# Alee08/multiagent-rl-rm

Hardware: AMD Instinct MI355X
Metric: env×agent steps/sec at 65,536 envs (1/2/4/8 GPU) + CPU-ref parity rate (higher is better)
Workload: dtype int32; 1 GPU; FrozenLake map1, 65,536 envs/GPU x 2 agents, built-in A->B->C RM (3-state RM), random actions; n_envs_per_gpu=65536, n_envs_total=65536, n_agents=2, rm_states=4, parallelism=dp1 (env shards, no data-path collective), dispatch=queue, windows=5

## Files before the change

include/rmx.h:

```cpp
#ifndef RMX_H
#define RMX_H

#include <stdint.h>
#include <stddef.h>

#ifdef __cplusplus
extern "C" {
#endif

#define RMX_ABI_VERSION 12

#define RMX_MAX_AGENTS 8
#define RMX_MAX_CELLS 4096
#define RMX_MAX_RM_STATES 255
#define RMX_MAX_EVENTS 255

#define RMX_OK 0
#define RMX_E_INVALID (-1)
#define RMX_E_HIP (-2)
#define RMX_E_ACTION (-3)
#define RMX_E_STATE (-4)
#define RMX_E_TRACE (-5)

#define RMX_DEVICE_HOST (-1)
// ... 106 lines not shown
int rmx_step_hashed(rmx_handle* h, uint64_t seed, int64_t t_global, int autoreset, void* hip_stream);

int rmx_fill_actions(rmx_handle* h, uint64_t seed, int64_t t0, int32_t T, int32_t* actions_dev,
                     void* hip_stream);

int rmx_rollout(rmx_handle* h, uint64_t seed, int64_t t0, int32_t T, float* reward_trace_dev,
                void* hip_stream);

int rmx_mdp_states(rmx_handle* h, int32_t agent, int64_t* n_states);
int rmx_mdp(rmx_handle* h, int32_t agent, int32_t fix_frozen_lake, int32_t* next_dev, float* reward_dev,
            uint8_t* done_dev, void* hip_stream);

int rmx_stats_device(rmx_handle* h, double* out_dev, void* hip_stream);
int rmx_stats_host(rmx_handle* h, double* out_host);
int rmx_stats_clear(rmx_handle* h, void* hip_stream);

int rmx_step_report(rmx_handle* h, const int32_t* actions_dev, int autoreset, double* stats_out_dev,
                    void* hip_stream);
int rmx_step_report_fused(const rmx_handle* h);

int rmx_step_seq(rmx_handle* h, const int32_t* actions_dev, int64_t action_stride, int32_t n_steps, int autoreset,
                 double* stats_out_dev, void* hip_stream);
int rmx_seq_packed(const rmx_handle* h);
int rmx_queue_counters(const rmx_handle* h, int64_t* out3);
#define RMX_QUEUE_INFO_N 7
#define RMX_QUEUE_UNUSED 0
#define RMX_QUEUE_READY 1
#define RMX_QUEUE_UNAVAILABLE 2
#define RMX_QUEUE_RETIRED 3
#define RMX_SEQ_NONE 0
#define RMX_SEQ_QUEUE 1
#define RMX_SEQ_STREAM_KERNEL 2
#define RMX_SEQ_STREAM_DISABLED 3
#define RMX_SEQ_STREAM_QUEUE 4
#define RMX_SEQ_HOST 5
int rmx_queue_info(const rmx_handle* h, int64_t* out, int32_t n);
int rmx_queue_timing(rmx_handle* h, int every);
int rmx_queue_times(const rmx_handle* h, uint64_t* stamps, int64_t cap, int64_t* n);
int rmx_code_object_check(const void* co, size_t bytes, int64_t* n_step_kernels, int64_t* n_refused, char* report,
                          size_t report_cap);

#define RMX_VARIANT_GENERIC 0
#define RMX_VARIANT_LANE_PER_AGENT 1
#define RMX_VARIANT_FAST 2
#define RMX_VARIANT_FAST_LANE_PER_AGENT 3
#define RMX_VARIANT_HOST 4
// ... 58 lines not shown
```

multiagent-rl-rm_amd/csrc/rmx_capi_create.cpp:

```cpp
#include <algorithm>
#include <cstdlib>
#include <cstring>
#include <exception>
#include <string>
#include <vector>

#include "rmx_handle.h"

using namespace rmx::capi;

namespace {

int validate(const rmx_config* c) {
  if (!c) return fail(RMX_E_INVALID, "config is NULL");
  const std::string msg = rmx::validate_config(*c);
  return msg.empty() ? RMX_OK : fail(RMX_E_INVALID, msg);
}

int create_host(const rmx_config* cfg, rmx_handle** out) {
  rmx_handle* h = new rmx_handle();
  h->host = new rmx::HostEngine();
  const std::string msg = h->host->init(*cfg);
  if (!msg.empty()) {
    delete h->host;
// ... 19 lines not shown
      mj *= M;
      const u128 v[2] = {mj, sj};
      for (int k = 0; k < 2; ++k)
        for (int q = 0; q < 4; ++q) w[j][k][q] = (uint32_t)(v[k] >> (32 * q));
    }
  }
};
const RsJumpTable rs_jump_table;

}

extern "C" {

struct CreateTables {
  std::vector<unsigned char> blob, fast_blob;
  std::vector<uint32_t> merged_tab;
  std::vector<float> disc;
  std::vector<uint16_t> free_cells;
};

static void create_env(rmx_handle* h, const rmx_config* cfg) {
  if (const char* qv = std::getenv("RMX_QUEUE")) h->seq.queue_off = std::strcmp(qv, "0") == 0;
  if (const char* pv = std::getenv("RMX_SEQ_PACKED")) h->seq.packed_off = std::strcmp(pv, "0") == 0;
  if (const char* b = std::getenv("RMX_BLOCK")) {
    int v = std::atoi(b);
    if (v == 64 || v == 128 || v == 256) h->block = v;
  }
#ifdef RMX_DIAG
  if (const char* d = std::getenv("RMX_DIAG_BITS")) h->diag = std::atoi(d);
#endif
  const bool rng_on = cfg->stochastic || cfg->random_starts;
  if (rng_on) h->rollout_layout = rmx::kLayoutThreadPerEnv;
  if (const char* l = std::getenv("RMX_LAYOUT")) {
    if (!std::strcmp(l, "tpe")) h->step_layout = h->rollout_layout = rmx::kLayoutThreadPerEnv;
    if (!std::strcmp(l, "lpe") && !rng_on) h->step_layout = h->rollout_layout = rmx::kLayoutLanePerAgent;
  }
}

static bool create_plan(rmx_handle* h, const rmx_config* cfg, CreateTables& tb) {
  const int A = cfg->n_agents;
  for (int a = 0; a < A; ++a) {
    h->init_q[a] = cfg->init_q[a];
    h->final_q[a] = cfg->final_q[a];
    h->start_x[a] = cfg->start_xy[2 * a];
    h->start_y[a] = cfg->start_xy[2 * a + 1];
  }
// ... 170 lines not shown
```

multiagent-rl-rm_amd/csrc/rmx_capi_seq.cpp:

```cpp
#include <algorithm>
#include <atomic>
#include <cstring>
#include <exception>

#include "rmx_handle.h"

using namespace rmx::capi;

static bool seq_packs(const rmx_handle* h) {
  const int tm = h->fast_tables;
  return !h->seq.packed_off && !h->seq.pk_failed && !h->seq.pk_refused && h->cfg.n_envs < kFastWaveStatsMinEnvs &&
         rmx::pk_bytes(h->cfg.n_agents, (size_t)h->cfg.n_envs) < ((size_t)1 << 31) && fast_applies(h) && !h->cfg.stochastic && !h->cfg.random_starts &&
         !h->buf.qrm_s && !h->fast_wave_stats && h->fast_skip == rmx::kSkipRare &&
         (tm == rmx::kTblMerged4 || tm == rmx::kTblMerged) && h->cfg.n_agents <= rmx::kFastMaxAgents;
}

static bool seq_pack_buffer(rmx_handle* h) {
  if (h->seq.d_pk) return true;
  if (hipMalloc(&h->seq.d_pk, rmx::pk_bytes(h->cfg.n_agents, (size_t)h->cfg.n_envs)) != hipSuccess) {
    (void)hipGetLastError();
    h->seq.d_pk = nullptr;
    h->seq.pk_failed = true;
    return false;
  }
  return true;
}

static bool record_seq(rmx_handle* h, const int32_t* actions, int64_t stride, int32_t K, int autoreset,
                       double* stats_out, bool fused, bool packed) {
  h->seq.window.resize((size_t)K);
  for (int32_t k = 0; k < K; ++k) {
    const int32_t* a = actions + (size_t)k * (size_t)stride;
    const bool rpt = fused && k == K - 1;
    rmx::FastParams fp = rpt ? report_fp(h, a, autoreset, stats_out) : step_fp(h, a, 0, 0, autoreset);
    if (packed) fp.pk_io = k == 0 ? rmx::kIoColsToPk : (k == K - 1 ? rmx::kIoPkToCols : rmx::kIoPkToPk);
    rmx::StepCapture cap{&h->seq.window[(size_t)k], false};
    rmx::tl_capture = &cap;
    (void)rmx::launch_step_fast(fp, 0, h->cfg.kind, nullptr);
    rmx::tl_capture = nullptr;
    if (!cap.ok) return false;
    if (packed && !std::strstr(h->seq.window[(size_t)k].symbol, "step_fast_kernel_win")) return false;
  }
  return true;
}

static std::atomic<uint64_t> g_seq_keys{0};
constexpr int32_t kSeqMaxSteps = 1 << 20;

static int step_seq(rmx_handle* h, const int32_t* actions_dev, int64_t action_stride, int32_t n_steps, int autoreset,
                    double* stats_out_dev, void* stream) {
  int rc = check_bound(h);
  if (rc) return rc;
  if (!actions_dev || n_steps <= 0 || action_stride < 0) return fail(RMX_E_INVALID, "bad rmx_step_seq arguments");
  if (h->host) {
    h->seq.dispatch = RMX_SEQ_HOST;
    for (int32_t k = 0; k < n_steps; ++k) h->host->step(actions_dev + (size_t)k * (size_t)action_stride, autoreset);
    if (stats_out_dev) std::memcpy(stats_out_dev, h->host->stats, sizeof(h->host->stats));
    return RMX_OK;
  }
  SYNC_END_OR_RETURN(h);
  HIP_TRY(hipSetDevice(h->device), "hipSetDevice");
  if ((rc = starts_current(h, stream))) return rc;
  hipStream_t st = as_stream(stream);
  const bool fused = stats_out_dev && report_fuses(h);
// ... 56 lines not shown
    HIP_TRY(reduce_stats(h, stats_out_dev, st), "stats launch");
    HIP_TRY(hipStreamSynchronize(st), "step sequence");
  }
  return RMX_OK;
}

extern "C" {

int rmx_step_seq(rmx_handle* h, const int32_t* actions_dev, int64_t action_stride, int32_t n_steps, int autoreset,
                 double* stats_out_dev, void* stream) {
  if (n_steps > kSeqMaxSteps) return fail(RMX_E_INVALID, "rmx_step_seq: more steps than one window takes");
  try {
    return step_seq(h, actions_dev, action_stride, n_steps, autoreset, stats_out_dev, stream);
  } catch (const std::exception& e) {
    if (h) h->seq.key = 0;
    return fail(RMX_E_HIP, std::string("rmx_step_seq: ") + e.what());
  }
}

int rmx_seq_packed(const rmx_handle* h) {
  return h && !h->host && h->seq.dispatch == RMX_SEQ_QUEUE && h->seq.key && h->seq.is_packed ? 1 : 0;
}

int rmx_queue_counters(const rmx_handle* h, int64_t* out3) {
  if (!h || !out3) return fail(RMX_E_INVALID, "bad rmx_queue_counters arguments");
  rmx::QueueInfo qi{0, 0, 0, 0, RMX_QUEUE_UNUSED};
  if (!h->host) rmx::queue_info(h->device, &qi);
  out3[0] = qi.windows;
  out3[1] = qi.uploads;
  out3[2] = qi.packets;
  return RMX_OK;
}

int rmx_queue_info(const rmx_handle* h, int64_t* out, int32_t n) {
  if (!h || !out || n < 0) return fail(RMX_E_INVALID, "bad rmx_queue_info arguments");
  rmx::QueueInfo qi{0, 0, 0, 0, RMX_QUEUE_UNUSED};
  if (!h->host) rmx::queue_info(h->device, &qi);
  const int64_t v[RMX_QUEUE_INFO_N] = {qi.windows,         qi.uploads,      qi.packets, qi.stream_windows, qi.state,
                                       h->seq.dispatch, h->seq.recordings};
  for (int32_t i = 0; i < n && i < RMX_QUEUE_INFO_N; ++i) out[i] = v[i];
  return RMX_OK;
}

int rmx_queue_timing(rmx_handle* h, int every) {
  if (!h || every < 0) return fail(RMX_E_INVALID, "bad rmx_queue_timing arguments");
  if (h->host) return RMX_OK;
// ... 29 lines not shown
```

multiagent-rl-rm_amd/csrc/rmx_fast.hip:

```cpp
#include <hip/hip_runtime.h>

#include <cstddef>
#include <cstdio>
#include <cstring>
#include <type_traits>
#include <stdint.h>

#include "rmx_device.h"
#include "rmx_internal.h"

namespace rmx {

namespace {

__device__ __forceinline__ __amdgpu_buffer_rsrc_t col_rsrc(const void* base, uint32_t bytes) {
  return __builtin_amdgcn_make_buffer_rsrc(const_cast<void*>(base), 0, (int)bytes, 0x00020000);
}
constexpr int kStoreAux = 16;
constexpr int kStoreAuxNT = 18;
__device__ __forceinline__ int32_t col_ld(__amdgpu_buffer_rsrc_t r, uint32_t lane_bytes, uint32_t sgpr_bytes) {
  return __builtin_amdgcn_raw_buffer_load_b32(r, lane_bytes, sgpr_bytes, 0);
}
#ifdef RMX_DIAG
__device__ __forceinline__ void col_st_d(__amdgpu_buffer_rsrc_t r, uint32_t lane_bytes, uint32_t sgpr_bytes, int32_t v,
// ... 553 lines not shown
    }
  }
  if (__any(live && nx.i > 0)) {
    if (live) rs_draws<CHAIN>(nx, row, kRsDrawsPerStep / 2, n, A);
  }
  if (any_rs) {
    uint32_t* cw = reinterpret_cast<uint32_t*>(lds + (tid >> 6) * (uint32_t)kRsWaveLds);
    cw[lane] = fc0;
    cw[lane + 64] = fc1;
    asm volatile("" ::: "memory");
    if (rs && live) {
      const uint16_t* cells = reinterpret_cast<const uint16_t*>(cw);
#pragma unroll
      for (int a = 0; a < A; ++a) {
        const int32_t c = (int32_t)cells[slot[a]];
        sx[a] = c % p.W;
        sy[a] = c / p.W;
      }
    }
  }
}


template <int KIND, int A, bool HASHED, int TBL, int QXB = 0, int SKIP = kSkipNone, bool RPT = false,
          int SLIP = 0>
__global__ void __launch_bounds__(256) step_fast_kernel(int32_t N_arg, int32_t blk_arg, const int32_t* x_arg,
                                                        const int32_t* y_arg, const int32_t* q_arg,
                                                        const uint32_t* f_arg, const int32_t* t_arg,
                                                        const int32_t* act_arg, FastParams p) {
  constexpr int IO = kIoCols;
#include "rmx_fast_step.inc"
}

template <int KIND, int A, int TBL, bool RPT, int IO>
__global__ void __launch_bounds__(256) step_fast_kernel_win(int32_t N_arg, int32_t blk_arg, const int32_t* x_arg,
                                                            const int32_t* y_arg, const int32_t* q_arg,
                                                            const uint32_t* f_arg, const int32_t* t_arg,
                                                            const int32_t* act_arg, FastParams p) {
  constexpr bool HASHED = false;
  constexpr int QXB = 0, SKIP = kSkipRare, SLIP = 0;
#include "rmx_fast_step.inc"
}

template <int KIND, int A, int TBL, int SLIP = 0>
__global__ void __launch_bounds__(256) rollout_fast_kernel(FastParams p, int32_t T, float* __restrict__ trace) {
  static_assert(TBL == kTblGlobal || TBL == kTblMerged || TBL == kTblLds || TBL == kTblMergedLds,
// ... 257 lines not shown
static void launch_rollout_k(const FastParams& p, int32_t T, float* trace, hipStream_t st) {
  const dim3 b((unsigned)p.block), g((unsigned)(((int64_t)p.N + p.block - 1) / p.block));
  switch (p.A) {
    case 1: launch_rollout_a<KIND, 1>(p, T, trace, g, b, st); break;
    case 2: launch_rollout_a<KIND, 2>(p, T, trace, g, b, st); break;
    case 3: launch_rollout_a<KIND, 3>(p, T, trace, g, b, st); break;
    default: launch_rollout_a<KIND, 4>(p, T, trace, g, b, st); break;
  }
}

hipError_t launch_rollout_fast(const FastParams& p, int kind, int32_t T, float* trace, hipStream_t st) {
  if (kind == RMX_FROZEN_LAKE)
    launch_rollout_k<RMX_FROZEN_LAKE>(p, T, trace, st);
  else
    launch_rollout_k<RMX_OFFICE_WORLD>(p, T, trace, st);
  return hipGetLastError();
}

thread_local StepCapture* tl_capture = nullptr;

static StepArgs step_args(const FastParams& p, uint32_t blk) {
  return StepArgs{p.N, (int32_t)blk, p.pos_x, p.pos_y, p.rm_q, p.flags, p.t, p.actions, p};
}

static void capture_launch(StepCapture* c, dim3 g, dim3 b, size_t lds, const StepArgs& a, const FastParams& p) {
  StepLaunch& L = *c->out;
  L.grid = g.x;
  L.block = b.x;
  L.lds = (uint32_t)lds;
  std::memset(&L.args, 0, sizeof(L.args));
  std::memcpy(&L.args, &a, offsetof(StepArgs, p));
  std::memcpy(&L.args.p, &p, sizeof(FastParams));
  c->ok = true;
}

template <int KIND, int A, bool HASHED, int TBL, int QXB = 0, int SKIP = kSkipNone, bool RPT = false, int SLIP = 0>
static void go_step(dim3 g, dim3 b, size_t lds, hipStream_t st, const FastParams& p) {
  const StepArgs a = step_args(p, b.x);
  if (StepCapture* c = tl_capture) {
    snprintf(c->out->symbol, sizeof(c->out->symbol),
             "_ZN3rmx16step_fast_kernelILi%dELi%dELb%dELi%dELi%dELi%dELb%dELi%dEEEviiPKiS2_S2_PKjS2_S2_NS_"
             "10FastParamsE.kd",
             KIND, A, (int)HASHED, TBL, QXB, SKIP, (int)RPT, SLIP);
    return capture_launch(c, g, b, lds, a, p);
  }
  hipLaunchKernelGGL((step_fast_kernel<KIND, A, HASHED, TBL, QXB, SKIP, RPT, SLIP>), g, b, lds, st, a.N, a.blk, a.pos_x,
                     a.pos_y, a.rm_q, a.flags, a.t, a.actions, a.p);
}

template <int KIND, int A, int TBL, bool RPT, int IO>
static void go_step_win(dim3 g, dim3 b, hipStream_t st, const FastParams& p) {
  const StepArgs a = step_args(p, b.x);
  if (StepCapture* c = tl_capture) {
    snprintf(c->out->symbol, sizeof(c->out->symbol),
             "_ZN3rmx20step_fast_kernel_winILi%dELi%dELi%dELb%dELi%dEEEviiPKiS2_S2_PKjS2_S2_NS_10FastParamsE.kd", KIND, A,
             TBL, (int)RPT, IO);
    return capture_launch(c, g, b, 0, a, p);
  }
  hipLaunchKernelGGL((step_fast_kernel_win<KIND, A, TBL, RPT, IO>), g, b, 0, st, a.N, a.blk, a.pos_x, a.pos_y, a.rm_q,
                     a.flags, a.t, a.actions, a.p);
}

template <int KIND, int A, int TBL>
static void launch_win(const FastParams& p, dim3 g, dim3 b, hipStream_t st) {
  switch (p.pk_io) {
    case kIoColsToPk: go_step_win<KIND, A, TBL, false, kIoColsToPk>(g, b, st, p); break;
    case kIoPkToPk: go_step_win<KIND, A, TBL, false, kIoPkToPk>(g, b, st, p); break;
    default:
      if (p.rpt_out)
        go_step_win<KIND, A, TBL, true, kIoPkToCols>(g, b, st, p);
      else
        go_step_win<KIND, A, TBL, false, kIoPkToCols>(g, b, st, p);
      break;
  }
}
// ... 94 lines not shown
```

multiagent-rl-rm_amd/csrc/rmx_fast_step.inc:

```
  constexpr bool QRM = QXB > 0;
  constexpr bool IN_PK = IO == kIoPkToPk || IO == kIoPkToCols, OUT_PK = IO == kIoColsToPk || IO == kIoPkToPk;
  static_assert(IO == kIoCols || ((TBL == kTblMerged || TBL == kTblMerged4) && !HASHED && QXB == 0 && SLIP == 0 &&
                                  SKIP == kSkipRare),
                "packed windows: the deterministic merged-table step (x, y, rm_q come out of table bytes)");
  static_assert(!(RPT && OUT_PK), "the report rides in a window's last packet");
  static_assert(TBL == kTblGlobal || TBL == kTblMerged || TBL == kTblMerged4, "step: global or merged tables");
  static_assert(!QRM || TBL == kTblGlobal, "QRM outputs need the move word's event (global tables)");
  constexpr bool M4 = TBL == kTblMerged4;
  constexpr bool MERGED = TBL == kTblMerged || M4;
  constexpr bool STATS_FIRST = KIND == RMX_FROZEN_LAKE && A <= 2;
  constexpr bool RNG = SLIP != 0, DRAW = (SLIP & kRngSlip) != 0;
  constexpr bool RSTART = (SLIP & kRngStarts) != 0 && KIND == RMX_FROZEN_LAKE;
  constexpr int SAUX = SKIP == kSkipRareNT ? kStoreAuxNT : kStoreAux;
  const auto st = [&](__amdgpu_buffer_rsrc_t r, uint32_t lane_bytes, uint32_t sgpr_bytes, int32_t v) {
#ifdef RMX_DIAG
    if (p.diag & 32) {
      __builtin_amdgcn_raw_buffer_store_b32(v, r, lane_bytes, sgpr_bytes, 0);
      return;
    }
#endif
    __builtin_amdgcn_raw_buffer_store_b32(v, r, lane_bytes, sgpr_bytes, SAUX);
  };
  extern __shared__ __attribute__((aligned(16))) unsigned char lds[];
  const int tid = threadIdx.x;
#ifdef RMX_DIAG
  uint64_t st_clk[kStamps] = {}, st_rt[kStamps] = {};
#endif
  STAMP(0);
  constexpr bool PRE = A >= 3;
  const int32_t N = PRE ? N_arg : p.N;
#ifdef RMX_DIAG
  uint32_t wg = blockIdx.x;
  if ((p.diag & 65536) && (gridDim.x & 7u) == 0) wg = (wg & 7u) * (gridDim.x >> 3) + (wg >> 3);
  const int32_t e_raw = (int32_t)(wg * blockDim.x) + tid;
#else
  const int32_t e_raw = (int32_t)blockIdx.x * (PRE ? blk_arg : (int32_t)blockDim.x) + tid;
#endif
  const bool live = e_raw < N;
  const int32_t e = live ? e_raw : N - 1;
  const uint32_t off = (uint32_t)e * 4u;
  const uint32_t col = (uint32_t)N * 4u;
  const uint32_t cols = col * (uint32_t)A;
  const auto r_x = col_rsrc(PRE ? x_arg : p.pos_x, cols), r_y = col_rsrc(PRE ? y_arg : p.pos_y, cols);
  const auto r_q = col_rsrc(PRE ? q_arg : p.rm_q, cols), r_f = col_rsrc(PRE ? f_arg : p.flags, cols);
  const auto r_t = col_rsrc(PRE ? t_arg : p.t, col);
  const auto r_act = col_rsrc(PRE ? act_arg : p.actions, cols), r_rew = col_rsrc(p.reward, cols);
  AgentIO s[A];
  AgentIO s0[A];
  int32_t t;
  if constexpr (!IN_PK) t = col_ld(r_t, off, 0);
  __amdgpu_buffer_rsrc_t r_ret;
  [[maybe_unused]] const auto r_pk = col_rsrc(p.pk, IO != kIoCols ? col * (uint32_t)(3 * A + 1) : 0u);
  if constexpr (IN_PK) {
    t = col_ld(r_pk, off, (uint32_t)pk_col_t(A) * col);
    r_ret = col_rsrc(p.ep_ret, cols);
#pragma unroll
    for (int a = 0; a < A; ++a) {
      const uint32_t cw = (uint32_t)col_ld(r_pk, off, (uint32_t)pk_col_cell(A, a) * col);
      s[a].x = (int32_t)pk_x(cw);
      s[a].y = (int32_t)pk_y(cw);
      s[a].q = (int32_t)pk_q(cw);
      s[a].f = (uint32_t)col_ld(r_pk, off, (uint32_t)pk_col_flags(A, a) * col);
      s[a].ret = __int_as_float(col_ld(r_pk, off, (uint32_t)pk_col_ret(A, a) * col));
      s[a].act = col_ld(r_act, off, a * col);
      s0[a] = s[a];
    }
  } else if constexpr (!PRE) {
    r_ret = col_rsrc(p.ep_ret, cols);
#pragma unroll
    for (int a = 0; a < A; ++a) {
      s[a].x = col_ld(r_x, off, a * col);
      s[a].y = col_ld(r_y, off, a * col);
      s[a].q = col_ld(r_q, off, a * col);
      s[a].f = (uint32_t)col_ld(r_f, off, a * col);
      s[a].ret = __int_as_float(col_ld(r_ret, off, a * col));
      s[a].act = HASHED ? hash_action(p.seed, p.t_global, p.n_global, p.env_offset + e, A, a) : col_ld(r_act, off, a * col);
      s0[a] = s[a];
    }
  } else {
#pragma unroll
    for (int a = 0; a < A; ++a) {
      s[a].x = col_ld(r_x, off, a * col);
      s[a].y = col_ld(r_y, off, a * col);
      s[a].q = col_ld(r_q, off, a * col);
      s[a].f = (uint32_t)col_ld(r_f, off, a * col);
      s[a].act = HASHED ? hash_action(p.seed, p.t_global, p.n_global, p.env_offset + e, A, a) : col_ld(r_act, off, a * col);
      if constexpr (KIND == RMX_FROZEN_LAKE) __builtin_amdgcn_sched_barrier(0);
    }
// ... 247 lines not shown
      LaneStats ls = {0.0, (int)done, 0, done ? t1 : 0};
      double rsum = 0.0;
#pragma unroll
      for (int a = 0; a < A; ++a) {
        rsum += (double)s[a].ret;
        ls.successes += done ? (int)o[a].succ : 0;
      }
      ls.ret = done ? rsum : 0.0;
      wave_flush_slot(p.slab, slot, ls, __any(done));
    } else if (done) {
      double rs = 0.0;
      uint32_t sc = 0;
#pragma unroll
      for (int a = 0; a < A; ++a) {
        rs += (double)s[a].ret;
        sc += o[a].succ;
      }
      env_stats_env(p, e, t1);
      env_stats_ret(p, e, rs, sc);
    }
  };
  if constexpr (STATS_FIRST) flush_stats();
  STAMP(6);
  if constexpr (OUT_PK) {
    if (live) {
      st(r_pk, off, (uint32_t)pk_col_t(A) * col, t1);
#pragma unroll
      for (int a = 0; a < A; ++a) {
        const uint32_t f1 = s[a].f | (done ? RMX_F_ENV_DONE : 0u);
        st(r_pk, off, (uint32_t)pk_col_cell(A, a) * col, (int32_t)pk_cell((uint32_t)s[a].x, (uint32_t)s[a].y, (uint32_t)s[a].q));
        st(r_pk, off, (uint32_t)pk_col_flags(A, a) * col, (int32_t)f1);
        if (IO == kIoColsToPk || __float_as_int(s[a].ret) != __float_as_int(s0[a].ret))
          st(r_pk, off, (uint32_t)pk_col_ret(A, a) * col, __float_as_int(s[a].ret));
      }
    } else {
      bad = 0;
    }
  } else if (live) {
    constexpr bool ALL = SKIP == kSkipNone || IO == kIoPkToCols;
    st(r_t, off, 0, t1);
    if (p.env_done) byte_st<SAUX>(p, (uint32_t)e, done);
#pragma unroll
    for (int a = 0; a < A; ++a) {
      const uint32_t f1 = s[a].f | (done ? RMX_F_ENV_DONE : 0u);
      st(r_x, off, a * col, s[a].x);
      st(r_y, off, a * col, s[a].y);
// ... 101 lines not shown
  if constexpr (!STATS_FIRST) flush_stats();
#ifdef RMX_DIAG
  }
  STAMP(8);
  if (p.stamps && (tid & 63) == 0) {
    unsigned long long* w = p.stamps + (((size_t)blockIdx.x * blockDim.x + tid) >> 6) * (2 * kStamps);
#pragma unroll
    for (int i = 0; i < kStamps; ++i) {
      w[i] = st_clk[i];
      w[kStamps + i] = st_rt[i];
    }
  }
#endif
  if constexpr (RPT) {
    double rs = 0.0;
    uint32_t sc = 0;
#pragma unroll
    for (int a = 0; a < A; ++a) {
      rs += (double)s[a].ret;
      sc += o[a].succ;
    }
    report_tail(p, rin, done, rs, sc, t1);
  }
```

multiagent-rl-rm_amd/csrc/rmx_handle.h:

```cpp
#pragma once
#include <hip/hip_runtime.h>

#include <chrono>
#include <string>
#include <vector>

#include "rmx_host.h"
#include "rmx_hoststep.h"
#include "rmx_internal.h"

struct rmx_handle {
  rmx_config cfg;
  rmx::HostEngine* host = nullptr;
  struct Seq {
    std::vector<rmx::StepLaunch> window;
    rmx::FastParams base;
    const int32_t* actions = nullptr;
    const double* out = nullptr;
    int64_t stride = 0;
    int32_t k = 0;
    int autoreset = -1;
    uint64_t key = 0;
    bool queue_off = false;
    bool packed_off = false;
    bool pk_failed = false;
    bool pk_refused = false;
    uint32_t* d_pk = nullptr;
    bool is_packed = false;
    int dispatch = RMX_SEQ_NONE;
    int64_t recordings = 0;
  } seq;
  int device = 0;
  int block = 256;
  int step_layout = rmx::kLayoutThreadPerEnv;
  int rollout_layout = rmx::kLayoutLanePerAgent;
  void* d_tables = nullptr;
  size_t tables_bytes = 0;
  int32_t off_cell = 0, off_ev = 0, off_nq = 0, off_rr = 0, off_sh = 0, off_qrm = 0;
  int32_t n_qrm[RMX_MAX_AGENTS]{}, enc_nq[RMX_MAX_AGENTS]{};
  float* d_disc = nullptr;
  double* d_slab = nullptr;
  int64_t n_waves = 0;
  double* d_stats = nullptr;
  uint32_t* d_err = nullptr;
  rmx_buffers buf{};
  bool bound = false;
  uint64_t base_seed = 123;
// ... 133 lines not shown
```

multiagent-rl-rm_amd/csrc/rmx_internal.h:

```cpp
#pragma once
#include <hip/hip_runtime.h>
#include <stdint.h>

#include <cmath>
#include <string>

#include "../../include/rmx.h"
#include "rmx_layout.h"
#include "rmx_learn.h"
#include "rmx_rules.h"

namespace rmx {

__host__ __device__ constexpr int32_t shuffle_stride(int32_t n) { return (n + 7) & ~7; }
__host__ __device__ constexpr int32_t rs_wave_lds(int32_t n) { return 256 * ((n + 3) >> 2) + 512; }
constexpr int kRsWaveLds = 512 + 8 * 64 * (16 + 8);
constexpr int kRsRowMax = 192;
constexpr int kRngSlip = 1, kRngStarts = 2, kRngFixedSeed = 4;
inline size_t start_cache_rng_off(int A, int64_t N) { return (4 * (size_t)((A + 1) / 2) * (size_t)N + 255) & ~(size_t)255; }
inline size_t start_cache_bytes(int A, int64_t N) { return start_cache_rng_off(A, N) + 32 * (size_t)N; }

template <typename P>
inline void slip_fill(P& p, const rmx_config& c) {
  bool uniform = true;
// ... 158 lines not shown
   X(slip_thr) X(slip_uniform) X(pad4) X(slip_pack) X(seed_scale) X(seed_env_stride) X(seed_episode_stride) \
   X(base_seed) X(rng) X(episode) X(slip) X(n_free) X(free_cells) X(start_ws) X(nx_rng) X(nx_idx) X(nx_ep) \
   X(rs_jump) X(rs_cells) X(rs_rng) X(rs_dirty) X(pad5) X(pk) X(pk_io) X(pad7)
#define RMX_FP_FIELD_BYTES(f) +sizeof(FastParams::f)
constexpr size_t kFastParamsFieldBytes = 0 RMX_FAST_PARAMS_FIELDS(RMX_FP_FIELD_BYTES);
#undef RMX_FP_FIELD_BYTES
static_assert(kFastParamsFieldBytes == sizeof(FastParams), "FastParams has implicit padding or an unlisted field");
constexpr int kStamps = 9;

hipError_t launch_step_fast(const FastParams& p, int hashed, int kind, hipStream_t st);

struct StepArgs {
  int32_t N, blk;
  const int32_t *pos_x, *pos_y, *rm_q;
  const uint32_t* flags;
  const int32_t* t;
  const int32_t* actions;
  FastParams p;
};
static_assert(sizeof(StepArgs) == 56 + sizeof(FastParams), "step_fast_kernel's parameter list: no padding");
struct StepLaunch {
  char symbol[160];
  uint32_t grid, block, lds;
  StepArgs args;
};
struct StepCapture {
  StepLaunch* out;
  bool ok;
};
extern thread_local StepCapture* tl_capture;
constexpr int kQueueStream = 1;
constexpr int kQueueUnused = RMX_QUEUE_UNUSED, kQueueReady = RMX_QUEUE_READY, kQueueUnavailable = RMX_QUEUE_UNAVAILABLE,
              kQueueRetired = RMX_QUEUE_RETIRED;
int queue_run(int device, const StepLaunch* L, int K, uint64_t key, std::string* err);
void queue_note_stream(int device);
struct QueueInfo {
  int64_t windows, uploads, packets, stream_windows;
  int state;
};
void queue_info(int device, QueueInfo* out);
void queue_set_timing(int device, int every);
int64_t queue_times(int device, uint64_t* out, int64_t cap);
int code_object_check(const void* co, size_t bytes, int64_t* n_step, int64_t* n_refused, std::string* first);
hipError_t launch_rollout_fast(const FastParams& p, int kind, int32_t T, float* trace, hipStream_t st);

constexpr uint32_t kSyncStep = 1, kSyncReset = 2, kSyncExit = 3;
constexpr int kSyncInlineActs = 15;
constexpr uint32_t kSyncInline = 1u << 3, kSyncAutoreset = 1u << 2, kSyncBadAct = 15u;
// ... 64 lines not shown
```

multiagent-rl-rm_amd/csrc/rmx_queue.cpp:

```cpp
#include <hip/hip_runtime.h>
#include <hsa/hsa.h>
#include <hsa/hsa_ext_amd.h>

#include <algorithm>
#include <atomic>
#include <chrono>
#include <cstdlib>
#include <cstring>
#include <mutex>
#include <string>
#include <unordered_map>
#include <vector>

#include "rmx_comd.h"
#include "rmx_internal.h"

extern "C" const char rmx_fast_co_begin[];
extern "C" const char rmx_fast_co_end[];

namespace rmx {
namespace {

constexpr uint32_t kQueueSize = 1024;
constexpr size_t kSlotAlign = 64;
// ... 17 lines not shown
  uint32_t kargs, group, priv;
};

struct DeviceQueue {
  std::mutex mu;
  int state = kQueueUnused;
  std::string err;
  std::string inject;
  hsa_agent_t agent{};
  hsa_code_object_reader_t reader{};
  hsa_executable_t exec{};
  hsa_queue_t* q = nullptr;
  hsa_signal_t done{};
  uint64_t tick_hz = 0;
  std::unordered_map<std::string, Kernel> kernels;
  char* kargs_dev = nullptr;
  size_t kargs_cap = 0;
  std::vector<unsigned char> kargs_img;
  size_t kargs_valid = 0;
  std::vector<unsigned char> scratch;
  std::atomic<int> fault{0};
  uint64_t last_key = 0;
  std::vector<hsa_kernel_dispatch_packet_t> built;
  int64_t windows = 0, uploads = 0, packets = 0, stream_windows = 0;
  int timing = 0;
  bool profiled = false;
  bool early = true;
  std::vector<hsa_signal_t> tsig;
  std::vector<uint64_t> times;
};

constexpr int kMaxDevices = 64;
DeviceQueue g_dev[kMaxDevices];

std::string hsa_msg(const char* what, hsa_status_t s) {
  const char* m = nullptr;
  hsa_status_string(s, &m);
  return std::string(what) + ": " + (m ? m : "hsa error") + " (" + std::to_string((int)s) + ")";
}

#define HSA_OR_FAIL(expr, what)           \
  do {                                    \
    hsa_status_t s_ = (expr);             \
    if (s_ != HSA_STATUS_SUCCESS) {       \
      d.err = hsa_msg(what, s_);          \
      return false;                       \
// ... 150 lines not shown
      d.kargs_cap = 0;
      *err = "rmx queue: kernarg allocation failed";
      return -1;
    }
    d.kargs_cap = bytes;
  }
  const size_t same = std::min(bytes, d.kargs_valid);
  size_t lo = 0, hi = bytes;
  while (lo < same && d.scratch[lo] == d.kargs_img[lo]) ++lo;
  if (bytes <= d.kargs_valid)
    while (hi > lo && d.scratch[hi - 1] == d.kargs_img[hi - 1]) --hi;
  if (lo < hi) {
    d.kargs_valid = std::min(d.kargs_valid, lo);
    if (hipMemcpy(d.kargs_dev + lo, d.scratch.data() + lo, hi - lo, hipMemcpyHostToDevice) != hipSuccess) {
      *err = "rmx queue: kernarg upload failed";
      return -1;
    }
    if (d.kargs_img.size() < hi) d.kargs_img.resize(hi);
    std::memcpy(d.kargs_img.data() + lo, d.scratch.data() + lo, hi - lo);
    d.kargs_valid = std::max(d.kargs_valid, hi);
    ++d.uploads;
  }
  d.built.assign((size_t)K, hsa_kernel_dispatch_packet_t{});
  for (int i = 0; i < K; ++i) {
    hsa_kernel_dispatch_packet_t& pk = d.built[(size_t)i];
    pk.workgroup_size_x = (uint16_t)L[i].block;
    pk.workgroup_size_y = 1;
    pk.workgroup_size_z = 1;
    pk.grid_size_x = L[i].grid * L[i].block;
    pk.grid_size_y = 1;
    pk.grid_size_z = 1;
    pk.private_segment_size = ks[i]->priv;
    pk.group_segment_size = ks[i]->group + L[i].lds;
    pk.kernel_object = ks[i]->object;
    pk.kernarg_address = d.kargs_dev + slot * i;
  }
  return 0;
}

int retire(DeviceQueue& d, const char* why, std::string* err) {
  if (d.q) (void)hsa_queue_inactivate(d.q);
  d.state = kQueueRetired;
  d.err = why;
  d.last_key = 0;
  *err = d.err;
  return -1;
}
// ... 59 lines not shown
  for (uint64_t j = 0; j < pad; ++j) {
    auto* bp = reinterpret_cast<hsa_barrier_and_packet_t*>(ring + ((w0 + j) & (size - 1)));
    std::memset(reinterpret_cast<char*>(bp) + 4, 0, sizeof(*bp) - 4);
    __atomic_store_n(reinterpret_cast<uint32_t*>(bp), (uint32_t)(HSA_PACKET_TYPE_BARRIER_AND << HSA_PACKET_HEADER_TYPE),
                     __ATOMIC_RELEASE);
  }
  if (pad) hsa_signal_store_screlease(q->doorbell_signal, (hsa_signal_value_t)(base - 1));
  ++d.windows;
  const int bell = d.early ? kBell : 0;
  for (int i = 0; i < K; ++i) {
    const uint64_t idx = base + (uint64_t)i;
    if (i > 0 && (idx & (size - 1)) == 0)
      hsa_signal_store_screlease(q->doorbell_signal, (hsa_signal_value_t)(idx - 1));
    for (uint32_t spin = 0; idx - hsa_queue_load_read_index_scacquire(q) >= size; ++spin) {
      if (d.fault.load()) return retire(d, "rmx queue: the queue faulted", err);
      if ((spin & 1023u) == 1023u && Clock::now() > deadline)
        return retire(d, "rmx queue: no ring room for a window's packets (the packet processor stalled)", err);
    }
    hsa_kernel_dispatch_packet_t* pk = ring + (idx & (size - 1));
    const hsa_kernel_dispatch_packet_t& b = d.built[(size_t)i];
    std::memcpy(reinterpret_cast<char*>(pk) + 4, reinterpret_cast<const char*>(&b) + 4, sizeof(b) - 4);
    pk->completion_signal = i == K - 1 ? d.done : n_timed && sig_of[(size_t)i] >= 0 ? d.tsig[(size_t)sig_of[(size_t)i]]
                                                                                   : hsa_signal_t{0};
    const uint16_t header = (uint16_t)((HSA_PACKET_TYPE_KERNEL_DISPATCH << HSA_PACKET_HEADER_TYPE) |
                                       (1 << HSA_PACKET_HEADER_BARRIER) |
                                       (HSA_FENCE_SCOPE_AGENT << HSA_PACKET_HEADER_SCACQUIRE_FENCE_SCOPE) |
                                       (HSA_FENCE_SCOPE_AGENT << HSA_PACKET_HEADER_SCRELEASE_FENCE_SCOPE));
    const uint16_t setup = 1 << HSA_KERNEL_DISPATCH_PACKET_SETUP_DIMENSIONS;
    __atomic_store_n(reinterpret_cast<uint32_t*>(pk), (uint32_t)header | ((uint32_t)setup << 16), __ATOMIC_RELEASE);
    ++d.packets;
    if (bell && i + 1 < K && (i == 0 || (i + 1) % bell == 0))
      hsa_signal_store_screlease(q->doorbell_signal, (hsa_signal_value_t)idx);
  }
  hsa_signal_store_screlease(q->doorbell_signal, (hsa_signal_value_t)(base + (uint64_t)K - 1));
  const double left = std::max(0.0, std::chrono::duration<double>(deadline - Clock::now()).count());
  const uint64_t timeout = (uint64_t)(left * (double)d.tick_hz);
  const hsa_signal_value_t v =
      hsa_signal_wait_scacquire(d.done, HSA_SIGNAL_CONDITION_LT, 1, timeout, HSA_WAIT_STATE_ACTIVE);
  if (d.fault.load()) return retire(d, "rmx queue: the queue faulted", err);
  if (v >= 1) return retire(d, "rmx queue: a window did not complete", err);
  if (n_timed) {
    d.times.resize(3 * (size_t)n_timed);
    for (int j = 0; j < n_timed; ++j) {
      hsa_amd_profiling_dispatch_time_t t{};
      const hsa_signal_t sg = j == n_timed - 1 ? d.done : d.tsig[(size_t)j];
      if (hsa_amd_profiling_get_dispatch_time(d.agent, sg, &t) != HSA_STATUS_SUCCESS) {
        d.times.clear();
        *err = "rmx queue: hsa_amd_profiling_get_dispatch_time failed";
        return -1;
      }
// ... 62 lines not shown
```

multiagent-rl-rm_amd/rmx/_capi.py:

```python
from __future__ import annotations

import ctypes as C
import importlib.util
import os

from .tables import CompiledTables

LIB_NAME = "librmx.so"
LIB_PATH = os.path.join(os.path.dirname(os.path.abspath(__file__)), LIB_NAME)

RMX_OK, RMX_E_INVALID, RMX_E_HIP, RMX_E_ACTION, RMX_E_STATE, RMX_E_TRACE = 0, -1, -2, -3, -4, -5
F_ACTIVE, F_FAIL, F_TERM, F_TRUNC, F_ENV_TERM, F_RM_TERM, F_ENV_DONE = 0x01, 0x02, 0x04, 0x08, 0x10, 0x20, 0x40
F_STEPS_SHIFT = 16
NSTATS = 4
STAT_SUM_RETURN, STAT_EPISODES, STAT_SUCCESSES, STAT_SUM_LENGTH = 0, 1, 2, 3

EXPORTS = (
    "rmx_abi_version", "rmx_last_error", "rmx_build_info", "rmx_create", "rmx_destroy", "rmx_bind", "rmx_reset",
    "rmx_step", "rmx_step_hashed", "rmx_fill_actions", "rmx_rollout", "rmx_stats_device", "rmx_stats_host",
    "rmx_stats_clear", "rmx_check_errors", "rmx_mdp_states", "rmx_mdp", "rmx_step_variant", "rmx_state_bytes",
    "rmx_get_state", "rmx_set_state", "rmx_step_report", "rmx_step_report_fused", "rmx_reset_sync", "rmx_step_sync",
    "rmx_step_sync_begin", "rmx_sync_wait", "rmx_sync_end", "rmx_step_seq", "rmx_queue_counters", "rmx_queue_info",
    "rmx_code_object_check", "rmx_device_count", "rmx_queue_timing", "rmx_queue_times", "rmx_step_info",
    "rmx_seq_packed", "rmx_learn_states", "rmx_learn_bind", "rmx_learn_step", "rmx_learn_step_policy",
    "rmx_learn_rng_bind", "rmx_learn_rng_seed", "rmx_learn_lambda_slots", "rmx_learn_lambda_bind",
    "rmx_learn_traces_clear", "rmx_learn_run", "rmx_learn_eps_bind", "rmx_learn_eps_decay",
)
LEARN_UPDATE, LEARN_BEST, LEARN_NUMPY = 1, 2, 4
LEARN_DYN_FIXED, LEARN_DYN_ENV = 0, 1
LEARN_RUN_MAX = 4096
SYNC_MAX_ENVS = 256
QUEUE_INFO_N = 7
QUEUE_STATES = ("unused", "ready", "unavailable", "retired")
SEQ_DISPATCH = ("none", "queue", "stream:kernel", "stream:disabled", "stream:queue", "host")
VARIANT_GENERIC, VARIANT_LANE_PER_AGENT, VARIANT_FAST, VARIANT_FAST_LANE_PER_AGENT, VARIANT_HOST = 0, 1, 2, 3, 4
STEP_INFO_N = 14
STEP_INFO_FIELDS = ("variant", "tables", "record_bytes", "merged_sections", "merged_bytes", "merged4_bytes",
                    "fast_blob_bytes", "generic_blob_bytes", "store_mode", "wave_stats", "block", "qrm_fast",
                    "seed_fixed", "rollout_layout")
VARIANT_NAMES = ("generic", "lane_per_agent", "fast", "fast_lpe", "host")
TABLE_MODES = ("none", "global", "merged", "merged4")
LAYOUTS = ("thread_per_env", "lane_per_agent")
DEVICE_HOST = -1


ABI_VERSION = 12

CSRC = os.path.join(os.path.dirname(os.path.dirname(os.path.abspath(__file__))), "csrc")
# ... 124 lines not shown
        "rmx_abi_version": (C.c_int, []),
        "rmx_device_count": (C.c_int, [C.POINTER(C.c_int32)]),
        "rmx_last_error": (C.c_char_p, []),
        "rmx_build_info": (C.c_char_p, []),
        "rmx_state_bytes": (C.c_int, [vp, C.POINTER(C.c_size_t)]),
        "rmx_get_state": (C.c_int, [vp, vp, C.c_size_t]),
        "rmx_set_state": (C.c_int, [vp, vp, C.c_size_t]),
        "rmx_create": (C.c_int, [C.POINTER(RmxConfig), C.POINTER(vp)]),
        "rmx_destroy": (None, [vp]),
        "rmx_bind": (C.c_int, [vp, C.POINTER(RmxBuffers)]),
        "rmx_reset": (C.c_int, [vp, vp, u64, vp]),
        "rmx_step": (C.c_int, [vp, vp, C.c_int, vp]),
        "rmx_step_hashed": (C.c_int, [vp, u64, i64, C.c_int, vp]),
        "rmx_fill_actions": (C.c_int, [vp, u64, i64, i32, vp, vp]),
        "rmx_rollout": (C.c_int, [vp, u64, i64, i32, vp, vp]),
        "rmx_stats_device": (C.c_int, [vp, vp, vp]),
        "rmx_stats_host": (C.c_int, [vp, C.POINTER(C.c_double)]),
        "rmx_stats_clear": (C.c_int, [vp, vp]),
        "rmx_check_errors": (C.c_int, [vp]),
        "rmx_step_variant": (C.c_int, [vp]),
        "rmx_step_report": (C.c_int, [vp, vp, C.c_int, vp, vp]),
        "rmx_step_report_fused": (C.c_int, [vp]),
        "rmx_seq_packed": (C.c_int, [vp]),
        "rmx_step_seq": (C.c_int, [vp, vp, C.c_int64, C.c_int32, C.c_int, vp, vp]),
        "rmx_queue_timing": (C.c_int, [vp, C.c_int]),
        "rmx_queue_times": (C.c_int, [vp, vp, C.c_int64, C.POINTER(C.c_int64)]),
        "rmx_queue_counters": (C.c_int, [vp, vp]),
        "rmx_queue_info": (C.c_int, [vp, vp, i32]),
        "rmx_step_info": (C.c_int, [vp, vp, i32]),
        "rmx_code_object_check": (C.c_int, [vp, C.c_size_t, C.POINTER(C.c_int64), C.POINTER(C.c_int64), C.c_char_p,
                                            C.c_size_t]),
        "rmx_mdp_states": (C.c_int, [vp, i32, C.POINTER(C.c_int64)]),
        "rmx_mdp": (C.c_int, [vp, i32, i32, vp, vp, vp, vp]),
        "rmx_reset_sync": (C.c_int, [vp, u64, C.POINTER(RmxBuffers), vp]),
        "rmx_step_sync": (C.c_int, [vp, vp, C.c_int, C.POINTER(RmxBuffers), vp]),
        "rmx_step_sync_begin": (C.c_int, [vp, vp, C.c_int, vp]),
        "rmx_sync_wait": (C.c_int, [vp, C.POINTER(RmxBuffers)]),
        "rmx_sync_end": (C.c_int, [vp]),
        "rmx_learn_states": (C.c_int, [vp, C.POINTER(C.c_int64)]),
        "rmx_learn_bind": (C.c_int, [vp, C.POINTER(RmxLearnConfig), vp, vp]),
        "rmx_learn_step": (C.c_int, [vp, vp, C.c_int, vp]),
        "rmx_learn_step_policy": (C.c_int, [vp, C.c_double, C.c_int, u64, i64, C.c_int, vp, vp]),
        "rmx_learn_run": (C.c_int, [vp, C.c_int32, C.c_double, C.c_int, u64, i64, vp, vp]),
        "rmx_learn_rng_bind": (C.c_int, [vp, vp]),
        "rmx_learn_rng_seed": (C.c_int, [vp, vp, vp]),
        "rmx_learn_lambda_slots": (C.c_int, [vp, C.POINTER(C.c_int32)]),
# ... 35 lines not shown
```

Before: 39.64 billion (env x agent)-steps/s.

## Skip agent-scope release fences between packed step-window dispatches

For packed multi-step queue windows, every dispatch packet except the last now uses no release fence scope instead of agent scope. Correctness is meant to rest on the kernel itself: it issues an s_waitcnt vmcnt(0) after its packed stores, and a static_assert limits this to store paths that are safe for the hand-off. The packed-input kernel also gets the packet pointer as a preloaded argument (passed through x_arg) for agent counts at or above a threshold, delaying setup of the ep_ret descriptor. Setting RMX_SEQ_RELEASE=1 restores full release fences. The aim is to cut per-dispatch cache writeback/flush cost between steps, at the risk of memory visibility bugs if any store escapes the explicit wait.

```diff
diff --git a/include/rmx.h b/include/rmx.h
--- a/include/rmx.h
+++ b/include/rmx.h
@@ -152,6 +152,7 @@
 int rmx_step_seq(rmx_handle* h, const int32_t* actions_dev, int64_t action_stride, int32_t n_steps, int autoreset,
                  double* stats_out_dev, void* hip_stream);
 int rmx_seq_packed(const rmx_handle* h);
+int rmx_seq_handoff(int32_t k, int32_t n_steps, int packed, int release_all);
 int rmx_queue_counters(const rmx_handle* h, int64_t* out3);
 #define RMX_QUEUE_INFO_N 7
 #define RMX_QUEUE_UNUSED 0
diff --git a/multiagent-rl-rm_amd/csrc/rmx_capi_create.cpp b/multiagent-rl-rm_amd/csrc/rmx_capi_create.cpp
--- a/multiagent-rl-rm_amd/csrc/rmx_capi_create.cpp
+++ b/multiagent-rl-rm_amd/csrc/rmx_capi_create.cpp
@@ -65,6 +65,7 @@
 static void create_env(rmx_handle* h, const rmx_config* cfg) {
   if (const char* qv = std::getenv("RMX_QUEUE")) h->seq.queue_off = std::strcmp(qv, "0") == 0;
   if (const char* pv = std::getenv("RMX_SEQ_PACKED")) h->seq.packed_off = std::strcmp(pv, "0") == 0;
+  if (const char* rv = std::getenv("RMX_SEQ_RELEASE")) h->seq.release_all = std::strcmp(rv, "1") == 0;
   if (const char* b = std::getenv("RMX_BLOCK")) {
     int v = std::atoi(b);
     if (v == 64 || v == 128 || v == 256) h->block = v;
diff --git a/multiagent-rl-rm_amd/csrc/rmx_capi_seq.cpp b/multiagent-rl-rm_amd/csrc/rmx_capi_seq.cpp
--- a/multiagent-rl-rm_amd/csrc/rmx_capi_seq.cpp
+++ b/multiagent-rl-rm_amd/csrc/rmx_capi_seq.cpp
@@ -40,6 +40,7 @@
     rmx::tl_capture = nullptr;
     if (!cap.ok) return false;
     if (packed && !std::strstr(h->seq.window[(size_t)k].symbol, "step_fast_kernel_win")) return false;
+    h->seq.window[(size_t)k].handoff = rmx::seq_handoff(k, K, packed, h->seq.release_all) ? 1u : 0u;
   }
   return true;
 }
@@ -142,6 +143,10 @@
   return h && !h->host && h->seq.dispatch == RMX_SEQ_QUEUE && h->seq.key && h->seq.is_packed ? 1 : 0;
 }
 
+int rmx_seq_handoff(int32_t k, int32_t n_steps, int packed, int release_all) {
+  return rmx::seq_handoff(k, n_steps, packed != 0, release_all != 0) ? 1 : 0;
+}
+
 int rmx_queue_counters(const rmx_handle* h, int64_t* out3) {
   if (!h || !out3) return fail(RMX_E_INVALID, "bad rmx_queue_counters arguments");
   rmx::QueueInfo qi{0, 0, 0, 0, RMX_QUEUE_UNUSED};
diff --git a/multiagent-rl-rm_amd/csrc/rmx_fast.hip b/multiagent-rl-rm_amd/csrc/rmx_fast.hip
--- a/multiagent-rl-rm_amd/csrc/rmx_fast.hip
+++ b/multiagent-rl-rm_amd/csrc/rmx_fast.hip
@@ -599,6 +599,8 @@
 }
 
 
+constexpr int kWinPreMinA = 3;
+
 template <int KIND, int A, bool HASHED, int TBL, int QXB = 0, int SKIP = kSkipNone, bool RPT = false,
           int SLIP = 0>
 __global__ void __launch_bounds__(256) step_fast_kernel(int32_t N_arg, int32_t blk_arg, const int32_t* x_arg,
@@ -902,12 +904,18 @@
 static StepArgs step_args(const FastParams& p, uint32_t blk) {
   return StepArgs{p.N, (int32_t)blk, p.pos_x, p.pos_y, p.rm_q, p.flags, p.t, p.actions, p};
 }
+static StepArgs step_args_win(const FastParams& p, uint32_t blk, int io) {
+  StepArgs a = step_args(p, blk);
+  if (io == kIoPkToPk || io == kIoPkToCols) a.pos_x = reinterpret_cast<const int32_t*>(p.pk);
+  return a;
+}
 
 static void capture_launch(StepCapture* c, dim3 g, dim3 b, size_t lds, const StepArgs& a, const FastParams& p) {
   StepLaunch& L = *c->out;
   L.grid = g.x;
   L.block = b.x;
   L.lds = (uint32_t)lds;
+  L.handoff = 0;
   std::memset(&L.args, 0, sizeof(L.args));
   std::memcpy(&L.args, &a, offsetof(StepArgs, p));
   std::memcpy(&L.args.p, &p, sizeof(FastParams));
@@ -930,7 +938,7 @@
 
 template <int KIND, int A, int TBL, bool RPT, int IO>
 static void go_step_win(dim3 g, dim3 b, hipStream_t st, const FastParams& p) {
-  const StepArgs a = step_args(p, b.x);
+  const StepArgs a = step_args_win(p, b.x, IO);
   if (StepCapture* c = tl_capture) {
     snprintf(c->out->symbol, sizeof(c->out->symbol),
              "_ZN3rmx20step_fast_kernel_winILi%dELi%dELi%dELb%dELi%dEEEviiPKiS2_S2_PKjS2_S2_NS_10FastParamsE.kd", KIND, A,
diff --git a/multiagent-rl-rm_amd/csrc/rmx_fast_step.inc b/multiagent-rl-rm_amd/csrc/rmx_fast_step.inc
--- a/multiagent-rl-rm_amd/csrc/rmx_fast_step.inc
+++ b/multiagent-rl-rm_amd/csrc/rmx_fast_step.inc
@@ -27,7 +27,8 @@
   uint64_t st_clk[kStamps] = {}, st_rt[kStamps] = {};
 #endif
   STAMP(0);
-  constexpr bool PRE = A >= 3;
+  constexpr bool PK_PRE = IN_PK && A >= kWinPreMinA;
+  constexpr bool PRE = A >= 3 || PK_PRE;
   const int32_t N = PRE ? N_arg : p.N;
 #ifdef RMX_DIAG
   uint32_t wg = blockIdx.x;
@@ -41,7 +42,7 @@
   const uint32_t off = (uint32_t)e * 4u;
   const uint32_t col = (uint32_t)N * 4u;
   const uint32_t cols = col * (uint32_t)A;
-  const auto r_x = col_rsrc(PRE ? x_arg : p.pos_x, cols), r_y = col_rsrc(PRE ? y_arg : p.pos_y, cols);
+  const auto r_x = col_rsrc(PRE && !PK_PRE ? x_arg : p.pos_x, cols), r_y = col_rsrc(PRE ? y_arg : p.pos_y, cols);
   const auto r_q = col_rsrc(PRE ? q_arg : p.rm_q, cols), r_f = col_rsrc(PRE ? f_arg : p.flags, cols);
   const auto r_t = col_rsrc(PRE ? t_arg : p.t, col);
   const auto r_act = col_rsrc(PRE ? act_arg : p.actions, cols), r_rew = col_rsrc(p.reward, cols);
@@ -50,10 +51,11 @@
   int32_t t;
   if constexpr (!IN_PK) t = col_ld(r_t, off, 0);
   __amdgpu_buffer_rsrc_t r_ret;
-  [[maybe_unused]] const auto r_pk = col_rsrc(p.pk, IO != kIoCols ? col * (uint32_t)(3 * A + 1) : 0u);
+  [[maybe_unused]] const auto r_pk =
+      col_rsrc(PK_PRE ? (const void*)x_arg : (const void*)p.pk, IO != kIoCols ? col * (uint32_t)(3 * A + 1) : 0u);
   if constexpr (IN_PK) {
     t = col_ld(r_pk, off, (uint32_t)pk_col_t(A) * col);
-    r_ret = col_rsrc(p.ep_ret, cols);
+    if constexpr (!PK_PRE) r_ret = col_rsrc(p.ep_ret, cols);
 #pragma unroll
     for (int a = 0; a < A; ++a) {
       const uint32_t cw = (uint32_t)col_ld(r_pk, off, (uint32_t)pk_col_cell(A, a) * col);
@@ -64,6 +66,10 @@
       s[a].ret = __int_as_float(col_ld(r_pk, off, (uint32_t)pk_col_ret(A, a) * col));
       s[a].act = col_ld(r_act, off, a * col);
       s0[a] = s[a];
+    }
+    if constexpr (PK_PRE) {
+      __builtin_amdgcn_sched_barrier(0);
+      r_ret = col_rsrc(p.ep_ret, cols);
     }
   } else if constexpr (!PRE) {
     r_ret = col_rsrc(p.ep_ret, cols);
@@ -357,6 +363,8 @@
   };
   if constexpr (STATS_FIRST) flush_stats();
   STAMP(6);
+  static_assert(!OUT_PK || (SAUX == kStoreAux && !QRM && !RNG && !RPT && IO != kIoCols),
+                "a hand-off packet stores through st() with sc1 and through agent-scope atomics only");
   if constexpr (OUT_PK) {
     if (live) {
       st(r_pk, off, (uint32_t)pk_col_t(A) * col, t1);
@@ -504,3 +512,4 @@
     }
     report_tail(p, rin, done, rs, sc, t1);
   }
+  if constexpr (OUT_PK) asm volatile("s_waitcnt vmcnt(0)" ::: "memory");
diff --git a/multiagent-rl-rm_amd/csrc/rmx_handle.h b/multiagent-rl-rm_amd/csrc/rmx_handle.h
--- a/multiagent-rl-rm_amd/csrc/rmx_handle.h
+++ b/multiagent-rl-rm_amd/csrc/rmx_handle.h
@@ -23,6 +23,7 @@
     uint64_t key = 0;
     bool queue_off = false;
     bool packed_off = false;
+    bool release_all = false;
     bool pk_failed = false;
     bool pk_refused = false;
     uint32_t* d_pk = nullptr;
diff --git a/multiagent-rl-rm_amd/csrc/rmx_internal.h b/multiagent-rl-rm_amd/csrc/rmx_internal.h
--- a/multiagent-rl-rm_amd/csrc/rmx_internal.h
+++ b/multiagent-rl-rm_amd/csrc/rmx_internal.h
@@ -204,8 +204,12 @@
 struct StepLaunch {
   char symbol[160];
   uint32_t grid, block, lds;
+  uint32_t handoff;
   StepArgs args;
 };
+constexpr bool seq_handoff(int32_t k, int32_t K, bool packed, bool release_all) {
+  return packed && !release_all && K >= 2 && k >= 0 && k < K - 1;
+}
 struct StepCapture {
   StepLaunch* out;
   bool ok;
diff --git a/multiagent-rl-rm_amd/csrc/rmx_queue.cpp b/multiagent-rl-rm_amd/csrc/rmx_queue.cpp
--- a/multiagent-rl-rm_amd/csrc/rmx_queue.cpp
+++ b/multiagent-rl-rm_amd/csrc/rmx_queue.cpp
@@ -63,6 +63,7 @@
   std::atomic<int> fault{0};
   uint64_t last_key = 0;
   std::vector<hsa_kernel_dispatch_packet_t> built;
+  std::vector<unsigned char> built_handoff;
   int64_t windows = 0, uploads = 0, packets = 0, stream_windows = 0;
   int timing = 0;
   bool profiled = false;
@@ -259,7 +260,9 @@
     ++d.uploads;
   }
   d.built.assign((size_t)K, hsa_kernel_dispatch_packet_t{});
+  d.built_handoff.assign((size_t)K, 0);
   for (int i = 0; i < K; ++i) {
+    d.built_handoff[(size_t)i] = L[i].handoff ? 1 : 0;
     hsa_kernel_dispatch_packet_t& pk = d.built[(size_t)i];
     pk.workgroup_size_x = (uint16_t)L[i].block;
     pk.workgroup_size_y = 1;
@@ -365,10 +368,11 @@
     std::memcpy(reinterpret_cast<char*>(pk) + 4, reinterpret_cast<const char*>(&b) + 4, sizeof(b) - 4);
     pk->completion_signal = i == K - 1 ? d.done : n_timed && sig_of[(size_t)i] >= 0 ? d.tsig[(size_t)sig_of[(size_t)i]]
                                                                                    : hsa_signal_t{0};
+    const int release = d.built_handoff[(size_t)i] && i + 1 < K ? HSA_FENCE_SCOPE_NONE : HSA_FENCE_SCOPE_AGENT;
     const uint16_t header = (uint16_t)((HSA_PACKET_TYPE_KERNEL_DISPATCH << HSA_PACKET_HEADER_TYPE) |
                                        (1 << HSA_PACKET_HEADER_BARRIER) |
                                        (HSA_FENCE_SCOPE_AGENT << HSA_PACKET_HEADER_SCACQUIRE_FENCE_SCOPE) |
-                                       (HSA_FENCE_SCOPE_AGENT << HSA_PACKET_HEADER_SCRELEASE_FENCE_SCOPE));
+                                       (release << HSA_PACKET_HEADER_SCRELEASE_FENCE_SCOPE));
     const uint16_t setup = 1 << HSA_KERNEL_DISPATCH_PACKET_SETUP_DIMENSIONS;
     __atomic_store_n(reinterpret_cast<uint32_t*>(pk), (uint32_t)header | ((uint32_t)setup << 16), __ATOMIC_RELEASE);
     ++d.packets;
diff --git a/multiagent-rl-rm_amd/rmx/_capi.py b/multiagent-rl-rm_amd/rmx/_capi.py
--- a/multiagent-rl-rm_amd/rmx/_capi.py
+++ b/multiagent-rl-rm_amd/rmx/_capi.py
@@ -22,8 +22,9 @@
     "rmx_get_state", "rmx_set_state", "rmx_step_report", "rmx_step_report_fused", "rmx_reset_sync", "rmx_step_sync",
     "rmx_step_sync_begin", "rmx_sync_wait", "rmx_sync_end", "rmx_step_seq", "rmx_queue_counters", "rmx_queue_info",
     "rmx_code_object_check", "rmx_device_count", "rmx_queue_timing", "rmx_queue_times", "rmx_step_info",
-    "rmx_seq_packed", "rmx_learn_states", "rmx_learn_bind", "rmx_learn_step", "rmx_learn_step_policy",
-    "rmx_learn_rng_bind", "rmx_learn_rng_seed", "rmx_learn_lambda_slots", "rmx_learn_lambda_bind",
+    "rmx_seq_packed", "rmx_seq_handoff", "rmx_learn_states", "rmx_learn_bind", "rmx_learn_step",
+    "rmx_learn_step_policy", "rmx_learn_rng_bind", "rmx_learn_rng_seed", "rmx_learn_lambda_slots",
+    "rmx_learn_lambda_bind",
     "rmx_learn_traces_clear", "rmx_learn_run", "rmx_learn_eps_bind", "rmx_learn_eps_decay",
 )
 LEARN_UPDATE, LEARN_BEST, LEARN_NUMPY = 1, 2, 4
@@ -194,6 +195,7 @@
         "rmx_step_report": (C.c_int, [vp, vp, C.c_int, vp, vp]),
         "rmx_step_report_fused": (C.c_int, [vp]),
         "rmx_seq_packed": (C.c_int, [vp]),
+        "rmx_seq_handoff": (C.c_int, [C.c_int32, C.c_int32, C.c_int, C.c_int]),
         "rmx_step_seq": (C.c_int, [vp, vp, C.c_int64, C.c_int32, C.c_int, vp, vp]),
         "rmx_queue_timing": (C.c_int, [vp, C.c_int]),
         "rmx_queue_times": (C.c_int, [vp, vp, C.c_int64, C.POINTER(C.c_int64)]),
```

Result: faster. 40.88 billion (env x agent)-steps/s (median of 6 runs) (+3.1%).
